# strukturag/libde265

Measured on NVIDIA H100. Metric: decoded frames/sec at 4K Main profile, bit-exact YUV; MC kernel HBM GB/s, higher is better.
Workload: dtype u8

## Files before the change

libde265_b200/csrc/engine.cu:

```cuda

#include <cuda_runtime.h>

#include <atomic>
#include <chrono>
#include <condition_variable>
#include <deque>
#include <exception>
#include <functional>
#include <mutex>
#include <string>
#include <sched.h>
#include <thread>
#include <cmath>
#include <cstdarg>
#include <cstdio>
#include <cstdlib>
#include <cstring>
#include <new>
#include <vector>

#include "b200hevc.h"
#include "dev_common.cuh"
#include "kernels_filter.cuh"
#include "kernels_mc.cuh"
// ... 204 lines not shown
    {
      std::lock_guard<std::mutex> lk(m);
      q.emplace_back(g, std::move(f));
      g->pending++;
    }
    cv.notify_one();
  }
  void wait(Group* g)
  {
    std::unique_lock<std::mutex> lk(m);
    done_cv.wait(lk, [g] { return g->pending == 0; });
  }
  void run(std::function<void()> f) { run(&own, std::move(f)); }
  void wait() { wait(&own); }
  ~HostPool()
  {
    {
      std::lock_guard<std::mutex> lk(m);
      stop = true;
    }
    cv.notify_all();
    for (auto& t : th) t.join();
  }
};

#define B200_MAX_CTX 12
#define B200_MAX_PHYS (B200_MAX_SLOTS + 32)
#define B200_STAGE_SETS 40
struct PipeCtx {
  cudaStream_t stream = nullptr;
  Surface scratch;
  uint8_t* sync_buf = nullptr;
  size_t sync_cap = 0;
  cudaEvent_t tail = nullptr;
};

struct SlotSync {
  cudaEvent_t written = nullptr;
  int writer = -1;
  cudaEvent_t read[B200_MAX_CTX] = {};
  bool read_pending[B200_MAX_CTX] = {};
};

#define PLAN_PU_PARTS 4
#define PLAN_INTRA_PARTS 8
struct IntraPart {
  uint32_t i0 = 0, i1 = 0, task_base = 0;
  std::vector<uint32_t> intra_idx, task_of, task_first, task_cell, diag_cnt, diag_off, fill;
};

struct AsyncState;
struct b200_engine {
  int device = 0;
  std::atomic<size_t> stage_cap_hint{0};
  std::mutex issue_m;
  AsyncState* async = nullptr;
  PipeCtx ctx[B200_MAX_CTX];
  StagingSet stage_pool[B200_STAGE_SETS];
  unsigned next_stage = 0;
  int n_ctx = 1, next_ctx = 0;
  Surface slot[B200_MAX_PHYS];
  SlotSync ssync[B200_MAX_PHYS];
  int lmap[B200_MAX_SLOTS];
  int owner[B200_MAX_PHYS];
  int last_owner[B200_MAX_PHYS];
  bool rename = true;
// ... 363 lines not shown
}

static int check_params(const b200_pic_params& p)
{
  if (p.width == 0 || p.height == 0) return set_err(B200_ERR_INVALID, "empty picture");
  if (p.log2_ctb_size < 4 || p.log2_ctb_size > 6) return set_err(B200_ERR_INVALID, "log2_ctb_size %d", p.log2_ctb_size);
  if (p.dst_slot >= B200_MAX_SLOTS) return set_err(B200_ERR_INVALID, "dst_slot %d", p.dst_slot);
  if (p.chroma_format_idc > 1) return set_err(B200_ERR_UNSUPPORTED, "chroma_format_idc %d: the device path implements 4:0:0 and 4:2:0", p.chroma_format_idc);
  if (p.bit_depth_luma < 8 || p.bit_depth_luma > 12 || p.bit_depth_chroma < 8 || p.bit_depth_chroma > 12)
    return set_err(B200_ERR_UNSUPPORTED, "bit depth %d/%d (8..12 supported)", p.bit_depth_luma, p.bit_depth_chroma);
  if ((p.bit_depth_luma > 8) != (p.bit_depth_chroma > 8)) return set_err(B200_ERR_UNSUPPORTED, "mixed 8-bit / high-bit-depth planes");
  if ((p.width & 7) || (p.height & 7)) return set_err(B200_ERR_INVALID, "picture size must be a multiple of the minimum CB size (8)");
  return B200_OK;
}

static DevPic make_devpic(const b200_pic_params& p, const Surface& cur, const Surface& out)
{
  DevPic d{};
  d.w = p.width; d.h = p.height;
  d.cw = cur.cw; d.ch = cur.ch;
  d.bd_y = p.bit_depth_luma; d.bd_c = p.bit_depth_chroma;
  d.log2ctb = p.log2_ctb_size;
  const int S = 1 << d.log2ctb;
  d.wctb = (p.width + S - 1) / S; d.hctb = (p.height + S - 1) / S;
  d.w4 = (p.width + 3) / 4; d.h4 = (p.height + 3) / 4;
  d.w8 = (p.width + 7) / 8; d.h8 = (p.height + 7) / 8;
  d.chroma = p.chroma_format_idc;
  d.cb_qp_off = p.pps_cb_qp_offset; d.cr_qp_off = p.pps_cr_qp_offset;
  d.flags = p.flags;
  for (int c = 0; c < 3; c++) { d.cur[c] = cur.plane[c]; d.out[c] = out.plane[c]; d.pitch[c] = cur.pitch[c]; }
  return d;
}

static size_t sync_sao_offset(const b200_pic_params& p)
{
  const size_t cw4 = p.chroma_format_idc ? (size_t)((p.width / 2 + 3) / 4) : 0, ch4 = p.chroma_format_idc ? (size_t)((p.height / 2 + 3) / 4) : 0;
  return (256 + (size_t)((p.width + 3) / 4) * ((p.height + 3) / 4) + 2 * cw4 * ch4 + 255) & ~(size_t)255;
}

template <typename P>
static int launch_picture(b200_engine* en, PipeCtx& cx, const PicLayout& L, const DevPic& dp, const RefTable& refs, const uint8_t* dbase)
{
  cudaStream_t st = cx.stream;
  const size_t* off = L.off;
  const int n_tiles = L.n_tiles;
  const bool run_deblock = L.run_deblock, run_sao = L.run_sao;
  if (en->timing) CU(cudaEventRecord(en->ev[1], st));
  if (n_tiles > 0) {
    if (sizeof(P) == 1 && !en->mc_legacy) {
      MctMaps maps;
      memset(&maps, 0, sizeof(maps));
      int n = 0;
      for (int i = 0; i < B200_MAX_SLOTS; i++) {
        maps.index_of_slot[i] = -1;
        if (!((L.ref_mask >> i) & 1) || !refs.plane[i][0] || !en->slot[en->lmap[i]].has_tm) continue;
        if (n == MCT_MAX_REFS) return set_err(B200_ERR_UNSUPPORTED, "picture references more than %d DPB slots", MCT_MAX_REFS);
        for (int k = 0; k < 2; k++) { maps.luma[k][n] = en->slot[en->lmap[i]].tm_luma[k]; maps.chroma[k][n] = en->slot[en->lmap[i]].tm_chroma[k]; }
        maps.index_of_slot[i] = (int8_t)n++;
        maps.valid_slots |= 1u << i;
      }
      const uint32_t* tw = (const uint32_t*)(dbase + off[12]);
      TL("mc", (k_inter_pred_tma<<<std::min(L.n_batches, en->num_sms * en->mc_ctas), MCT_CTA_THREADS, sizeof(MctShared), st>>>(
                   dp, maps, (const b200_pu*)(dbase + off[0]), (const b200_weight_entry*)(dbase + off[1]), tw, tw + n_tiles, L.n_batches)));
    } else if (sizeof(P) == 1)
      k_inter_pred8<<<std::min((n_tiles + MC8_UNITS_PER_CTA - 1) / MC8_UNITS_PER_CTA, en->num_sms * 5), MC8_WARPS * 32, 0, st>>>(dp, refs, (const b200_pu*)(dbase + off[0]), (const b200_weight_entry*)(dbase + off[1]),
                                                         (const uint32_t*)(dbase + off[12]), n_tiles);
    else
      k_inter_pred<P><<<(n_tiles + 3) / 4, 128, 0, st>>>(dp, refs, (const b200_pu*)(dbase + off[0]), (const b200_weight_entry*)(dbase + off[1]),
                                                           (const uint32_t*)(dbase + off[12]), n_tiles);
    en->launches++;
  }
  if (en->timing) CU(cudaEventRecord(en->ev[2], st));
  if ((L.n_a > 0 || L.n_b > 0) && L.params.stop_after_stage != B200_STAGE_INTER_PRED) {
    ReconArgs ra;
    ra.tus = (const b200_tu*)(dbase + off[2]);
    ra.coeffs = (const b200_coeff*)(dbase + off[5]);
    ra.scaling = L.has_scaling ? dbase + off[11] : nullptr;
    ra.ticket = (unsigned int*)cx.sync_buf;
    ra.region = en->region;
    ra.poll_ns = en->poll_ns;
    ra.err = en->intra_err;
    ra.err_host = en->intra_err_host;
    ra.spin_limit_ns = en->spin_limit_ns;
    const size_t cw4 = (size_t)((dp.cw + 3) / 4), ch4 = (size_t)((dp.ch + 3) / 4);
    ra.pend[0] = cx.sync_buf + 256;
    ra.pend[1] = ra.pend[0] + (size_t)dp.w4 * dp.h4;
    ra.pend[2] = ra.pend[1] + cw4 * ch4;
    ra.pend_w[0] = dp.w4;
    ra.pend_w[1] = ra.pend_w[2] = (int)cw4;
    ra.mark_list = nullptr;
    ra.n_mark = 0;
    if (L.n_b > 0) CU(cudaMemsetAsync(cx.sync_buf, 0, 256 + (size_t)dp.w4 * dp.h4 + 2 * cw4 * ch4, st));
    if (L.n_a > 0) {
      ra.list = (const uint32_t*)(dbase + off[3]);
      ra.n_list = L.n_a;
      ra.n_listw = L.n_aw;
      ra.n_list8 = L.n_a8;
      if (L.n_b > 0) {
        ra.mark_list = (const uint32_t*)(dbase + off[4]);
        ra.n_mark = L.n_b;
      }
      const int items = L.n_aw + (L.n_a8 + 3) / 4 + (L.n_a - L.n_aw - L.n_a8 + 31) / 32;
      TL("residual", (k_residual<P><<<std::min((items + RC_WARPS - 1) / RC_WARPS, en->num_sms * 4), RC_THREADS, 0, st>>>(dp, ra)));
      en->launches++;
    }
    ra.trace = nullptr;
    if (L.n_b > 0) {
      unsigned long long* trace_dev = nullptr;
      const char* trace_path = getenv("B200_TRACE_INTRA");
      if (trace_path && L.n_task > 0) {
        CU(cudaMalloc(&trace_dev, sizeof(unsigned long long) * RC_TRACE_WORDS * (size_t)L.n_task));
        CU(cudaMemsetAsync(trace_dev, 0, sizeof(unsigned long long) * RC_TRACE_WORDS * (size_t)L.n_task, st));
        ra.trace = trace_dev;
      }
      ra.list = (const uint32_t*)(dbase + off[4]);
      ra.n_list = L.n_b;
      if (L.n_a == 0) {
        TL("mark", (k_mark_pending<<<(L.n_b + 255) / 256, 256, 0, st>>>(ra)));
        en->launches++;
      }
      ra.task_start = (const uint32_t*)(dbase + off[13]);
      ra.n_task = L.n_task;
      int grid = (L.n_task + RC_WARPS - 1) / RC_WARPS;
      const bool background = L.ref_mask == 0 && en->n_ctx > 1;
      int cap = background ? (en->intra_i_grid ? en->intra_i_grid : en->num_sms) : en->num_sms * en->intra_ctas;
// ... 6 lines not shown
        std::vector<unsigned long long> h(RC_TRACE_WORDS * (size_t)L.n_task);
        std::vector<uint32_t> tasks((size_t)L.n_task + 1 + (size_t)L.n_b);
        CU(cudaStreamSynchronize(st));
        CU(cudaMemcpy(h.data(), trace_dev, h.size() * sizeof(unsigned long long), cudaMemcpyDeviceToHost));
        CU(cudaMemcpy(tasks.data(), ra.task_start, ((size_t)L.n_task + 1) * sizeof(uint32_t), cudaMemcpyDeviceToHost));
        CU(cudaMemcpy(tasks.data() + L.n_task + 1, ra.list, (size_t)L.n_b * sizeof(uint32_t), cudaMemcpyDeviceToHost));
        cudaFree(trace_dev);
        if (FILE* f = fopen(trace_path, "ab")) {
          const unsigned long long n[2] = {(unsigned long long)L.n_task, (unsigned long long)L.n_b};
          fwrite(n, sizeof(n), 1, f);
          fwrite(h.data(), sizeof(unsigned long long), h.size(), f);
          fwrite(tasks.data(), sizeof(uint32_t), tasks.size(), f);
          fclose(f);
        }
      }
    }
  }
  if (en->timing) CU(cudaEventRecord(en->ev[3], st));
  FilterArgs fa;
  fa.bs_map = dbase + off[8];
  fa.qp_map = (const int8_t*)(dbase + off[9]);
  fa.nofilt_map = dbase + off[10];
  fa.slices = (const b200_slice_info*)(dbase + off[6]);
  fa.ctbs = (const b200_ctb_info*)(dbase + off[7]);
  if (run_deblock) {
    const int nseg = ((dp.w4 + 1) / 2) * dp.h4 > dp.w4 * ((dp.h4 + 1) / 2) ? ((dp.w4 + 1) / 2) * dp.h4 : dp.w4 * ((dp.h4 + 1) / 2);
    dim3 grid((nseg + 127) / 128, dp.chroma ? 2 : 1);
    TL("deblock_v", (k_deblock<P, true><<<grid, 128, 0, st>>>(dp, fa)));
    TL("deblock_h", (k_deblock<P, false><<<grid, 128, 0, st>>>(dp, fa)));
    en->launches += 2;
  }
  if (en->timing) CU(cudaEventRecord(en->ev[4], st));
  if (run_sao) {
    uint16_t* avail = (uint16_t*)(cx.sync_buf + sync_sao_offset(L.params));
    fa.sao_avail = avail;
    const bool sao8 = sizeof(P) == 1 && dp.log2ctb >= 5 && !en->sao_legacy;
    if (!sao8) {
      TL("sao_prep", (k_sao_prep<<<(2 * dp.wctb * dp.hctb + 127) / 128, 128, 0, st>>>(dp, fa, avail)));
      en->launches++;
    }
    dim3 grid((dp.w / 8 + 127) / 128, dp.h, dp.chroma ? 3 : 1);
    if (sao8) {
      Sao8Layout lay;
      lay.n_ctb = dp.wctb * dp.hctb;
      const int S = 1 << dp.log2ctb, rows_l = (32 >> (dp.log2ctb - 4)) * SAO8_R, rows_c = (32 >> (dp.log2ctb - 5)) * SAO8_R;
      lay.ipl = (S + rows_l - 1) / rows_l;
      lay.ipc = dp.chroma ? (S / 2 + rows_c - 1) / rows_c : 0;
      const int items = lay.n_ctb * (lay.ipl + 2 * lay.ipc);
      TL("sao", (k_sao8<<<(items + SAO8_WARPS - 1) / SAO8_WARPS, SAO8_WARPS * 32, 0, st>>>(dp, fa, lay)));
    } else {
      TL("sao", (k_sao<P><<<grid, 128, 0, st>>>(dp, fa)));
    }
    en->launches++;
  }
  if (en->timing) CU(cudaEventRecord(en->ev[5], st));
  CU(cudaGetLastError());
  return B200_OK;
}

static const int k_raw_sections[10] = {0, 1, 2, 5, 6, 7, 8, 9, 10, 11};
static const int k_list_sections[4] = {3, 4, 12, 13};

static int plan_begin(b200_engine* en, const b200_picture* pic, PicLayout* L, size_t* cap_total)
{
  const b200_pic_params& p = pic->params;
  int rc = check_params(p);
  if (rc) return rc;
// ... 662 lines not shown
  RefTable refs;
  memset(&refs, 0, sizeof(refs));
  for (int i = 0; i < B200_MAX_SLOTS; i++) {
    if (i == p.dst_slot || en->lmap[i] < 0) continue;
    const Surface& s = en->slot[en->lmap[i]];
    if (s.valid && s.w == p.width && s.h == p.height && s.chroma == p.chroma_format_idc && s.bd_y == p.bit_depth_luma && s.bd_c == p.bit_depth_chroma)
      for (int c = 0; c < 3; c++) refs.plane[i][c] = s.plane[c];
  }
  {
    const uint64_t geom = (uint64_t)p.width | ((uint64_t)p.height << 16) | ((uint64_t)p.chroma_format_idc << 32) |
                          ((uint64_t)bytes_per_sample(p.bit_depth_luma) << 34) | ((uint64_t)bytes_per_sample(p.bit_depth_chroma) << 36);
    if (en->pool_geom && en->pool_geom != geom) {
      for (int c = 0; c < B200_MAX_CTX; c++) CU(cudaStreamSynchronize(en->ctx[c].stream));
      for (int ph = 0; ph < B200_MAX_PHYS; ph++)
        if (en->owner[ph] < 0 && en->slot[ph].plane[0] && !same_geometry(en->slot[ph], p)) surface_free(en->slot[ph]);
    }
    en->pool_geom = geom;
  }
  int dst_phys = phys_for_write(en, p.dst_slot, k, p);
  if (dst_phys < 0) {
    return set_err(B200_ERR_NOMEM, "no free picture surface");
  }
  Surface& dst = en->slot[dst_phys];
  int rc = surface_ensure(dst, p, cx.stream);
  if (rc) return rc;
  Surface* cur = &dst;
  if (L.run_sao) {
    rc = surface_ensure(cx.scratch, p, cx.stream);
    if (rc) return rc;
    cur = &cx.scratch;
  }
  {
    const size_t n_ctb = (size_t)((p.width + (1 << p.log2_ctb_size) - 1) >> p.log2_ctb_size) * ((p.height + (1 << p.log2_ctb_size) - 1) >> p.log2_ctb_size);
    const size_t need = sync_sao_offset(p) + 2 * n_ctb * sizeof(uint16_t);
    if (cx.sync_cap < need) {
      if (cx.sync_buf) { CU(cudaStreamSynchronize(cx.stream)); cudaFree(cx.sync_buf); }
      cx.sync_buf = nullptr;
      CU(cudaMalloc(&cx.sync_buf, need));
      cx.sync_cap = need;
    }
  }
  cudaStream_t st = cx.stream;
  en->ev = en->timing ? &en->tev[(size_t)(en->tcount % TIMING_RING) * 7] : nullptr;
  if (en->timing) CU(cudaEventRecord(en->ev[0], st));
  if (upload_from && L.direct) {
    for (int i : k_raw_sections)
      if (L.raw_sz[i]) CU(cudaMemcpyAsync(dbase + L.off[i], L.raw_src[i], L.raw_sz[i], cudaMemcpyHostToDevice, st));
    if (L.total > L.raw_total) CU(cudaMemcpyAsync(dbase + L.raw_total, upload_from + L.raw_total, L.total - L.raw_total, cudaMemcpyHostToDevice, st));
  } else if (upload_from) {
    CU(cudaMemcpyAsync(dbase, upload_from, L.total, cudaMemcpyHostToDevice, st));
  }
  if (prof) tseg[1] = now();
  rc = order_before(en, k, L, dst_phys);
  if (rc) return rc;
  if (prof) tseg[2] = now();
  const DevPic dp = make_devpic(p, *cur, dst);
  if (p.bit_depth_luma > 8) rc = launch_picture<uint16_t>(en, cx, L, dp, refs, dbase);
  else rc = launch_picture<uint8_t>(en, cx, L, dp, refs, dbase);
  if (rc) return rc;
  if (prof) tseg[3] = now();
  if (en->tl_path) tl_begin(en, st, "extend", L.params.poc, k);
  launch_extend_borders(dst, st);
  if (en->tl_path) tl_end(en, st);
  en->launches++;
  CU(cudaGetLastError());
  if (en->timing) { CU(cudaEventRecord(en->ev[6], st)); en->tcount++; }
  rc = order_after(en, k, L, dst_phys);
  if (rc) return rc;
  dst.valid = true;
  if (prof) {
    tseg[4] = now();
// ... 548 lines not shown
```

libde265_b200/csrc/kernels_recon.cuh:

```cuda
#pragma once
#include "dev_common.cuh"
#include "kernels_residual.cuh"

#define RC_WARPS 8
#define RC_THREADS (RC_WARPS * 32)
#define RC_GSTRIDE 34
#define RC_TILE_STRIDE 40
#define RC_BLK (33 * RC_TILE_STRIDE + 8)
#define RC_FULL 0xffffffffu
#define RC_TRACE_WORDS 8

struct ReconArgs {
  const b200_tu* tus;
  const uint32_t* list;
  int n_list;
  int poll_ns;
  int region;
  int n_listw, n_list8;
  const uint32_t* task_start;
  int n_task;
  const b200_coeff* coeffs;
  const uint8_t* scaling;
  unsigned int* ticket;
  unsigned long long* trace;
  uint8_t* pend[3];
  int pend_w[3];
  const uint32_t* mark_list;
  int n_mark;
  unsigned int* err;
  unsigned int* err_host;
  unsigned long long spin_limit_ns;
};

struct ResidualSmem {
  int16_t coef[RC_WARPS][32 * RC_GSTRIDE];
  int16_t g[RC_WARPS][32 * RC_GSTRIDE];
  ResTables tb;
};

template <typename P>
struct IntraSmem {
  P blk[RC_WARPS][RC_BLK];
  int16_t coef[RC_WARPS][32 * RC_GSTRIDE];
  int16_t g[RC_WARPS][32 * RC_GSTRIDE];
  res_t res[RC_WARPS][32 * 32];
  P border[RC_WARPS][2][4 * 32 + 4];
  b200_tu tu_s[RC_WARPS][16];
  ResTables tb;
};

template <typename P, bool TO_RES>
__device__ void tu_residual(const b200_tu& tu, const b200_coeff* co, const uint8_t* __restrict__ scaling, P* dst, int dstride, res_t* res,
                            int bd, int16_t* coefT, int16_t* g, const ResTables& tb, int lane)
{
  const int log2 = tu.log2_size, nT = 1 << log2, n = tu.n_coeff;
  const int flags = tu.flags;
  const bool special = flags & (B200_TU_BYPASS | B200_TU_TSKIP);
  const Dequant dq = dequant_setup(tu, scaling, bd);
  int max_row = 0, max_col = 0;
// ... 272 lines not shown
      if (bfilt) {
        if (mode == 26 && x == 0) v = clip_bd(B(1) + ((B(-1 - y) - B(0)) >> 1), bd);
        if (mode == 10 && y == 0) v = clip_bd(B(-1) + ((B(1 + x) - B(0)) >> 1), bd);
      }
      px[p] = v;
    }
  }
  __syncwarp();
#pragma unroll
  for (int p = 0; p < NP; p++) {
    const int o = lane + 32 * p, x = o & (nT - 1), y = (o >> LOG2) & (nT - 1);
    if (o < nT * nT) {
      int v = px[p];
      if (res) v = clip_bd(v + res[o], bd);
      dst[x + y * ts] = (P)v;
    }
  }
  __syncwarp();
}

__device__ __forceinline__ bool intra_fast_ok(const b200_tu& tu)
{
  const int g = 1 << (tu.log2_size - 2);
  const uint64_t need = ((1ull << g) - 1) | (1ull << B200_AVAIL_CORNER_BIT) | (((1ull << g) - 1) << B200_AVAIL_TOP_BIT0);
  if ((tu.avail & need) != need) return false;
  if (g == 2) {
    const unsigned bl = (unsigned)(tu.avail >> 2) & 3, tr = (unsigned)(tu.avail >> (B200_AVAIL_TOP_BIT0 + 2)) & 3;
    if (bl == 2 || tr == 2) return false;
  }
  return true;
}

template <typename P>
__device__ void tu_intra_large(const b200_tu& tu, const P* gsrc, int gstride, P* dst, int bd, int bd_luma, uint32_t pic_flags, bool filter_plane,
                               P* b0mem, P* b1mem, int lane)
{
  const int log2 = tu.log2_size, nT = 1 << log2, mode = tu.intra_mode, cidx = tu.cidx, dstride = nT;
  const uint64_t avail = tu.avail;
  P* b0 = b0mem + 2 * 32 + 2;
  P* b1 = b1mem + 2 * 32 + 2;
  const int total = 4 * nT + 1;
  {
    constexpr int MAXC = 5;
    int v[MAXC];
    bool av[MAXC];
#pragma unroll
    for (int c5 = 0; c5 < MAXC; c5++) {
      const int s = 32 * c5 + lane, i = s - 2 * nT;
      av[c5] = false;
      v[c5] = 0;
      if (s < total) {
        const P* addr;
        if (i < 0) { const int r = -i - 1; av[c5] = (avail >> (r >> 2)) & 1; addr = gsrc - 1 + r * gstride; }
        else if (i == 0) { av[c5] = (avail >> B200_AVAIL_CORNER_BIT) & 1; addr = gsrc - 1 - gstride; }
        else { const int c = i - 1; av[c5] = (avail >> (B200_AVAIL_TOP_BIT0 + (c >> 2))) & 1; addr = gsrc + c - gstride; }
        if (av[c5]) v[c5] = (int)__ldcg(addr);
      }
    }
    int first_val = 1 << (bd - 1);
    bool any = false;
#pragma unroll
    for (int c5 = 0; c5 < MAXC; c5++) {
      const unsigned m = __ballot_sync(0xffffffffu, av[c5]);
      if (!any && m) { first_val = __shfl_sync(0xffffffffu, v[c5], __ffs(m) - 1); any = true; }
    }
    if (!any) {
      for (int s = lane; s < total; s += 32) b0[s - 2 * nT] = (P)(1 << (bd - 1));
    } else {
      int carry = first_val;
#pragma unroll
      for (int c5 = 0; c5 < MAXC; c5++) {
        if (32 * c5 < total) {
          const int s = 32 * c5 + lane, i = s - 2 * nT;
          const unsigned m = __ballot_sync(0xffffffffu, av[c5]);
          const unsigned below = m & ((2u << lane) - 1u);
          const int src = below ? 31 - __clz(below) : 0;
          const int sv = __shfl_sync(0xffffffffu, v[c5], src);
          const int outv = below ? sv : carry;
          if (s < total) b0[i] = (P)outv;
          carry = __shfl_sync(0xffffffffu, outv, 31);
        }
      }
    }
  }
  __syncwarp();
  const P* bsrc = b0;
  if (filter_plane && mode != 1) {
    const int d = min(abs(mode - 26), abs(mode - 10));
    const bool filt = d > ((nT == 8) ? 7 : (nT == 16) ? 1 : 0);
    if (filt) {
      const bool strong = (pic_flags & B200_PIC_STRONG_INTRA_SMOOTHING) && cidx == 0 && nT == 32 &&
// ... 47 lines not shown
    for (int s = lane; s <= 3 * nT; s += 32) {
      const int x = s - nT;
      const bool w = (x >= 0) ? (x <= nT || angle >= 0) : (project && x >= last);
      const int idx = (x >= 0) ? sgn * x : -sgn * ((x * inv + 128) >> 8);
      if (w) ref[x] = bsrc[idx];
    }
    __syncwarp();
    const bool bfilt = (cidx == 0 && nT < 32 && !(tu.flags & B200_TU_NO_BOUNDARY_FILTER) && (mode == 26 || mode == 10));
    for (int o = lane; o < nT * nT; o += 32) {
      const int x = o & (nT - 1), y = o >> log2;
      const int a = vert ? y : x, b = vert ? x : y;
      const int idx = ((a + 1) * angle) >> 5, fact = ((a + 1) * angle) & 31;
      int v = fact ? ((32 - fact) * (int)ref[b + idx + 1] + fact * (int)ref[b + idx + 2] + 16) >> 5 : (int)ref[b + idx + 1];
      if (bfilt) {
        if (mode == 26 && x == 0) v = clip_bd((int)bsrc[1] + (((int)bsrc[-1 - y] - (int)bsrc[0]) >> 1), bd);
        if (mode == 10 && y == 0) v = clip_bd((int)bsrc[-1] + (((int)bsrc[1 + x] - (int)bsrc[0]) >> 1), bd);
      }
      dst[x + y * dstride] = (P)v;
    }
  }
  __syncwarp();
}

template <typename P>
__device__ __forceinline__ void block_store(const P* blk, uint8_t* plane, int pitch, int x, int y, int nT, int lane)
{
  const int upr = nT * (int)sizeof(P) / 4;
  for (int o = lane; o < nT * upr; o += 32) {
    const int r = o / upr, u = o % upr;
    *reinterpret_cast<uint32_t*>(plane + (size_t)(y + r) * pitch + (size_t)x * sizeof(P) + 4 * u) = reinterpret_cast<const uint32_t*>(blk + r * nT)[u];
  }
}

template <typename P>
__global__ void __launch_bounds__(RC_THREADS) k_residual(DevPic pic, ReconArgs args)
{
  __shared__ ResidualSmem sm;
  const int tid = threadIdx.x, warp = tid >> 5, lane = tid & 31;
  for (int i = tid; i < (int)(sizeof(ResTables) / 4); i += RC_THREADS) reinterpret_cast<uint32_t*>(&sm.tb)[i] = reinterpret_cast<const uint32_t*>(&c_res)[i];
  for (int i = blockIdx.x * RC_THREADS + tid; i < args.n_mark; i += gridDim.x * RC_THREADS) {
    const b200_tu tu = args.tus[args.mark_list[i]];
    const int c = tu.cidx, n4u = 1 << (tu.log2_size - 2);
    uint8_t* p = args.pend[c] + (tu.y >> 2) * args.pend_w[c] + (tu.x >> 2);
    for (int j = 0; j < n4u; j++)
      for (int k = 0; k < n4u; k++) p[j * args.pend_w[c] + k] = 1;
  }
  __syncthreads();
  const int n4 = args.n_list - args.n_listw - args.n_list8;
  const int Ww = args.n_listw, W8 = (args.n_list8 + 3) >> 2, W4 = (n4 + 31) >> 5;
  uint32_t* scratch = reinterpret_cast<uint32_t*>(sm.coef[warp]);
  for (int wi = blockIdx.x * RC_WARPS + warp; wi < Ww + W8 + W4; wi += gridDim.x * RC_WARPS) {
    if (wi < Ww) {
      const b200_tu tu = args.tus[args.list[wi]];
      const int c = tu.cidx, nT = 1 << tu.log2_size;
      P* dst = row_ptr<P>(pic.cur[c], pic.pitch[c], tu.y) + tu.x;
      const int dstride = pic.pitch[c] / (int)sizeof(P);
      if (tu.flags & B200_TU_PCM) {
        for (int i = lane; i < tu.n_coeff; i += 32) {
          const b200_coeff co = args.coeffs[tu.coeff_off + i];
          dst[(co.pos & (nT - 1)) + (co.pos >> tu.log2_size) * dstride] = (P)(uint16_t)co.level;
        }
      } else {
        tu_residual<P, false>(tu, args.coeffs + tu.coeff_off, args.scaling, dst, dstride, nullptr, c ? pic.bd_c : pic.bd_y, sm.coef[warp], sm.g[warp],
                              sm.tb, lane);
      }
    } else if (wi < Ww + W8) {
// ... 16 lines not shown
                            sm.tb);
      }
    }
    __syncwarp();
  }
}

__global__ void k_mark_pending(ReconArgs args)
{
  const int idx = blockIdx.x * blockDim.x + threadIdx.x;
  if (idx >= args.n_list) return;
  const b200_tu tu = args.tus[args.list[idx]];
  const int c = tu.cidx, n4 = 1 << (tu.log2_size - 2);
  uint8_t* p = args.pend[c] + (tu.y >> 2) * args.pend_w[c] + (tu.x >> 2);
  for (int j = 0; j < n4; j++)
    for (int i = 0; i < n4; i++) p[j * args.pend_w[c] + i] = 1;
}

__device__ __forceinline__ void dep_units_of(const b200_tu& tu, int rx, int ry, int span, unsigned& left, bool& corner, unsigned& top)
{
  const int half = 1 << (tu.log2_size - 1);
  const int ux0 = (tu.x - rx) >> 2, uy0 = (tu.y - ry) >> 2;
  const uint64_t avail = tu.avail;
  const unsigned gm = (half >= 32) ? 0xffffffffu : ((1u << half) - 1u), sm = (1u << span) - 1u;
  const bool cb = (avail >> B200_AVAIL_CORNER_BIT) & 1;
  if (ux0 == 0) {
    left |= (((unsigned)avail & gm) << uy0) & sm;
    if (cb) { if (uy0 == 0) corner = true; else left |= 1u << (uy0 - 1); }
  } else if (uy0 == 0 && cb) {
    top |= 1u << (ux0 - 1);
  }
  if (uy0 == 0) top |= (((unsigned)(avail >> B200_AVAIL_TOP_BIT0) & gm) << ux0) & sm;
}

__device__ __forceinline__ unsigned ld_acquire_u8(const uint8_t* p)
{
  unsigned v;
  asm volatile("ld.acquire.gpu.global.u8 %0, [%1];" : "=r"(v) : "l"(p) : "memory");
  return v;
}
__device__ __forceinline__ void st_relaxed_u8(uint8_t* p, unsigned v) { asm volatile("st.relaxed.gpu.global.u8 [%0], %1;" ::"l"(p), "r"(v) : "memory"); }

template <typename P>
__global__ void __launch_bounds__(RC_THREADS, 3) k_intra(DevPic pic, ReconArgs args)
{
  extern __shared__ __align__(16) uint8_t smem_raw[];
  IntraSmem<P>& sm = *reinterpret_cast<IntraSmem<P>*>(smem_raw);
  const int tid = threadIdx.x, warp = tid >> 5, lane = tid & 31;
  for (int i = tid; i < (int)(sizeof(ResTables) / 4); i += RC_THREADS) reinterpret_cast<uint32_t*>(&sm.tb)[i] = reinterpret_cast<const uint32_t*>(&c_res)[i];
  __syncthreads();
  b200_tu* tus = sm.tu_s[warp];
  res_t* res = sm.res[warp];
  P* blk = sm.blk[warp];
  for (;;) {
    unsigned t = 0;
    if (lane == 0) t = atomicAdd(args.ticket, 1u);
    t = __shfl_sync(RC_FULL, t, 0);
    if (t >= (unsigned)args.n_task) return;
    unsigned tr_c = 0;
    auto tr_time = [&](int w) {
      if (args.trace && lane == 0) {
        unsigned long long g;
        asm volatile("mov.u64 %0, %%globaltimer;" : "=l"(g));
        args.trace[(unsigned long long)RC_TRACE_WORDS * t + w] = g;
      }
    };
    auto tr_cycles = [&](int w) {
      if (args.trace && lane == 0) {
        const unsigned c = (unsigned)clock();
        if (w >= 0) args.trace[(unsigned long long)RC_TRACE_WORDS * t + w] += c - tr_c;
        tr_c = c;
      }
    };
    tr_time(0);
    tr_cycles(-1);
    const uint32_t first = args.task_start[t], count = min(args.task_start[t + 1] - first, 16u);
    if (lane < (int)count) tus[lane] = args.tus[args.list[first + lane]];
    __syncwarp();
    const b200_tu tu0 = tus[0];
    const int G0 = args.region >> (tu0.cidx ? 1 : 0);
    const bool region = (1 << tu0.log2_size) <= min(G0, 8);
    unsigned seg_starts;
    {
      const int mc = (lane < (int)count) ? tus[lane].cidx : -1, pc = (lane > 0 && lane < (int)count) ? tus[lane - 1].cidx : -1;
      seg_starts = __ballot_sync(RC_FULL, lane < (int)count && (lane == 0 || mc != pc));
    }
    {
      const bool mine = lane < (int)count;
      const b200_tu& mytu = tus[mine ? lane : 0];
      const int l2 = mytu.log2_size, sz = mine ? 1 << (2 * l2) : 0;
      const int mybd = mytu.cidx ? pic.bd_c : pic.bd_y;
      int incl = sz;
#pragma unroll
      for (int d = 1; d < 16; d <<= 1) {
        const int up = __shfl_up_sync(RC_FULL, incl, d);
        if (lane >= d) incl += up;
      }
      const int my_rbase = incl - sz;
      const bool cbf = mine && (mytu.flags & B200_TU_CBF);
      const unsigned m8 = __ballot_sync(RC_FULL, cbf && l2 == 3), mw = __ballot_sync(RC_FULL, cbf && l2 > 3);
      uint32_t* scratch = reinterpret_cast<uint32_t*>(sm.coef[warp]);
      if (cbf && l2 == 2) res4_lane<P, true>(mytu, args.coeffs + mytu.coeff_off, args.scaling, nullptr, 0, res + my_rbase, mybd, scratch, lane, sm.tb);
      __syncwarp();
      for (unsigned rem = m8; rem;) {
        const int q = lane >> 3;
        const unsigned idx = __fns(rem, 0, q + 1);
        const bool active = idx < 32u;
        const b200_tu& tu = tus[active ? idx : 0];
        const int rb = __shfl_sync(RC_FULL, my_rbase, active ? idx : 0);
        res8_quarter<P, true>(active, tu, args.coeffs + tu.coeff_off, args.scaling, nullptr, 0, res + rb, tu.cidx ? pic.bd_c : pic.bd_y, scratch + q * 64,
                              lane & 7, sm.tb);
#pragma unroll
        for (int k = 0; k < 4; k++) rem &= rem - 1;
      }
      for (unsigned rem = mw; rem; rem &= rem - 1) {
        const int idx = __ffs(rem) - 1;
        const b200_tu& tu = tus[idx];
        const int rb = __shfl_sync(RC_FULL, my_rbase, idx);
        tu_residual<P, true>(tu, args.coeffs + tu.coeff_off, args.scaling, nullptr, 0, res + rb, tu.cidx ? pic.bd_c : pic.bd_y, sm.coef[warp], sm.g[warp],
                             sm.tb, lane);
      }
    }
    tr_cycles(3);
    for (unsigned ss = seg_starts; ss; ss &= ss - 1) {
      const int s0 = __ffs(ss) - 1, s1 = (ss & (ss - 1)) ? __ffs(ss & (ss - 1)) - 1 : (int)count;
      const b200_tu& ts0 = tus[s0];
      const int c = ts0.cidx, G = args.region >> (c ? 1 : 0);
      const int rx = region ? ts0.x & ~(G - 1) : ts0.x, ry = region ? ts0.y & ~(G - 1) : ts0.y;
      const int span = region ? (2 * G) >> 2 : (1 << ts0.log2_size) >> 1;
      unsigned left = 0, top = 0;
      bool corner = false;
      if (lane >= s0 && lane < s1) dep_units_of(tus[lane], rx, ry, span, left, corner, top);
      left = __reduce_or_sync(RC_FULL, left);
      top = __reduce_or_sync(RC_FULL, top);
      corner = __any_sync(RC_FULL, corner);
      const int pw = args.pend_w[c];
      const uint8_t* pend = args.pend[c] + (ry >> 2) * pw + (rx >> 2);
      const uint8_t* f = nullptr;
      if (lane < span) { if ((left >> lane) & 1) f = pend + lane * pw - 1; }
      else if (lane == span) { if (corner) f = pend - pw - 1; }
      else if (lane - span - 1 < span) { if ((top >> (lane - span - 1)) & 1) f = pend - pw + (lane - span - 1); }
      const uint8_t* f2 = nullptr;
      if (span == 16 && lane == 0 && ((top >> 15) & 1)) f2 = pend - pw + 15;
      unsigned ns = 32, spins = 0;
      unsigned long long t_wait0 = 0;
      for (;;) {
        const bool busy = (f && ld_acquire_u8(f)) || (f2 && ld_acquire_u8(f2));
        if (!__any_sync(RC_FULL, busy)) break;
        __nanosleep(ns);
        if (ns < (unsigned)args.poll_ns) ns *= 2;
        else if ((++spins & 63u) == 0) {
          unsigned long long now;
          asm volatile("mov.u64 %0, %%globaltimer;" : "=l"(now));
          if (!t_wait0) t_wait0 = now;
          bool give_up = now - t_wait0 > args.spin_limit_ns || *(volatile unsigned int*)args.err != 0;
          give_up = __shfl_sync(RC_FULL, give_up, 0);
          if (give_up) {
            if (lane == 0) {
              atomicCAS(args.err, 0u, t + 1);
              *(volatile unsigned int*)args.err_host = t + 1;
              __threadfence_system();
            }
            break;
          }
        }
      }
    }
    __syncwarp();
    tr_time(1);
    tr_cycles(4);

    if (!region) {
      const int c = tu0.cidx, bd = c ? pic.bd_c : pic.bd_y;
      const bool filter_plane = !(pic.flags & B200_PIC_INTRA_SMOOTHING_OFF) && (c == 0 || pic.chroma == 3);
      const int nT = 1 << tu0.log2_size;
      const int gstride = pic.pitch[c] / (int)sizeof(P);
      const P* gsrc = row_ptr<P>(pic.cur[c], pic.pitch[c], tu0.y) + tu0.x;
      tu_intra_large<P>(tu0, gsrc, gstride, blk, bd, pic.bd_y, pic.flags, filter_plane, sm.border[warp][0], sm.border[warp][1], lane);
      if (tu0.flags & B200_TU_CBF) {
        for (int o = lane; o < nT * nT; o += 32) blk[o] = (P)clip_bd((int)blk[o] + res[o], bd);
        __syncwarp();
      }
      tr_cycles(6);
      block_store<P>(blk, pic.cur[c], pic.pitch[c], tu0.x, tu0.y, nT, lane);
    } else {
      int rbase = 0;
      for (unsigned ss = seg_starts; ss; ss &= ss - 1) {
        const int s0 = __ffs(ss) - 1, s1 = (ss & (ss - 1)) ? __ffs(ss & (ss - 1)) - 1 : (int)count;
        const b200_tu& ts0 = tus[s0];
        const int c = ts0.cidx, bd = c ? pic.bd_c : pic.bd_y, G = args.region >> (c ? 1 : 0);
        const int rx = ts0.x & ~(G - 1), ry = ts0.y & ~(G - 1);
        const bool filter_plane = !(pic.flags & B200_PIC_INTRA_SMOOTHING_OFF) && (c == 0 || pic.chroma == 3);
        const int pwid = c ? pic.cw : pic.w, phei = c ? pic.ch : pic.h;
        int covered = 0;
        for (int i = s0; i < s1; i++) covered += 1 << (2 * tus[i].log2_size);
        const int TS = RC_TILE_STRIDE;
        P* tile = blk + TS + 4;
        const int gw = min(G, pwid - rx), gh = min(G, phei - ry);
        const bool full = (gw == G) && (gh == G);
        tr_cycles(-1);
        const bool interior = covered < gw * gh;
        constexpr int NW = 2 * (int)sizeof(P);
        const int wpr = G * (int)sizeof(P) / 4;
        uint32_t in_w[NW];
        if (interior && full) {
#pragma unroll
          for (int k = 0; k < NW; k++) {
            const int o = lane + 32 * k;
            if (o < G * wpr) in_w[k] = __ldcg(reinterpret_cast<const uint32_t*>(row_ptr<P>(pic.cur[c], pic.pitch[c], ry + o / wpr) + rx) + o % wpr);
          }
        }
        const int xt0 = lane - 1, xt1 = lane + 31;
        const bool top0 = ry > 0 && xt0 < 2 * G && rx + xt0 >= 0 && rx + xt0 < pwid;
        const bool top1 = ry > 0 && xt1 < 2 * G && rx + xt1 < pwid;
        const bool left = rx > 0 && lane < 2 * G && ry + lane < phei;
        P top_s0, top_s1, left_s;
        if (top0) top_s0 = __ldcg(row_ptr<P>(pic.cur[c], pic.pitch[c], ry - 1) + rx + xt0);
        if (top1) top_s1 = __ldcg(row_ptr<P>(pic.cur[c], pic.pitch[c], ry - 1) + rx + xt1);
        if (left) left_s = __ldcg(row_ptr<P>(pic.cur[c], pic.pitch[c], ry + lane) + rx - 1);
        if (interior && full) {
#pragma unroll
          for (int k = 0; k < NW; k++) {
            const int o = lane + 32 * k;
            if (o < G * wpr) reinterpret_cast<uint32_t*>(tile + (o / wpr) * TS)[o % wpr] = in_w[k];
          }
        } else if (interior) {
          for (int o = lane; o < gw * gh; o += 32) {
            const int x = o % gw, y = o / gw;
            tile[y * TS + x] = __ldcg(row_ptr<P>(pic.cur[c], pic.pitch[c], ry + y) + rx + x);
          }
        }
        if (top0) tile[-TS + xt0] = top_s0;
        if (top1) tile[-TS + xt1] = top_s1;
        if (left) tile[lane * TS - 1] = left_s;
        __syncwarp();
        tr_cycles(5);
        for (int i = s0; i < s1; i++) {
          const b200_tu& tu = tus[i];
          P* tdst = tile + (tu.y - ry) * TS + (tu.x - rx);
          const res_t* tres = (tu.flags & B200_TU_CBF) ? res + rbase : nullptr;
          if (!intra_fast_ok(tu)) tu_intra_small<P>(tu, tdst, TS, bd, filter_plane, tres, lane);
          else if (tu.log2_size == 2) tu_intra_fast<P, 2>(tu, tdst, TS, bd, filter_plane, tres, lane);
          else tu_intra_fast<P, 3>(tu, tdst, TS, bd, filter_plane, tres, lane);
          rbase += 1 << (2 * tu.log2_size);
        }
        tr_cycles(6);
        if (full) {
          const int wpr = G * (int)sizeof(P) / 4;
          for (int o = lane; o < G * wpr; o += 32) {
            const int y = o / wpr, u = o % wpr;
            reinterpret_cast<uint32_t*>(row_ptr<P>(pic.cur[c], pic.pitch[c], ry + y) + rx)[u] = reinterpret_cast<const uint32_t*>(tile + y * TS)[u];
          }
        } else {
          for (int o = lane; o < gw * gh; o += 32) {
            const int x = o % gw, y = o / gw;
            row_ptr<P>(pic.cur[c], pic.pitch[c], ry + y)[rx + x] = tile[y * TS + x];
          }
        }
        __syncwarp();
      }
    }
    __syncwarp();
    if (lane < (int)count) {
      asm volatile("fence.release.gpu;" ::: "memory");
      const b200_tu& tu = tus[lane];
      const int n4 = 1 << (tu.log2_size - 2), pw = args.pend_w[tu.cidx];
      uint8_t* pend = args.pend[tu.cidx] + (tu.y >> 2) * pw + (tu.x >> 2);
      for (int j = 0; j < n4; j++)
        for (int i = 0; i < n4; i++) st_relaxed_u8(pend + j * pw + i, 0);
    }
    __syncwarp();
    tr_time(2);
    if (args.trace && lane == 0)
      args.trace[(unsigned long long)RC_TRACE_WORDS * t + 7] = count | ((unsigned long long)tu0.cidx << 8) | ((unsigned long long)tu0.log2_size << 16);
  }
}
```

Measured before the change: 2884.

## Replace per-TU pending-flag clears with tagged edge mailboxes in intra wavefront

Intra-prediction warps used to poll byte pending flags with acquire loads and clear them after each TU with a release fence. Now each finished block publishes its bottom row and right column as tagged 64-bit words into per-region mailboxes, so a dependent warp takes its neighbour samples straight from the mailbox once the tag matches. This removes the flag-clear and fence path and the re-read of neighbours from the picture. The tile interior is fetched with cp.async, which can overlap the wait. The cost is a larger sync buffer, extra stores for the edge data, and a periodic full memset when the tag wraps; correctness now depends on the tag and layout bookkeeping.

```diff
diff --git a/libde265_b200/csrc/engine.cu b/libde265_b200/csrc/engine.cu
--- a/libde265_b200/csrc/engine.cu
+++ b/libde265_b200/csrc/engine.cu
@@ -260,6 +260,7 @@
   Surface scratch;
   uint8_t* sync_buf = nullptr;
   size_t sync_cap = 0;
+  uint32_t tag = 0;
   cudaEvent_t tail = nullptr;
 };
 
@@ -689,10 +690,38 @@
   return d;
 }
 
-static size_t sync_sao_offset(const b200_pic_params& p)
-{
-  const size_t cw4 = p.chroma_format_idc ? (size_t)((p.width / 2 + 3) / 4) : 0, ch4 = p.chroma_format_idc ? (size_t)((p.height / 2 + 3) / 4) : 0;
-  return (256 + (size_t)((p.width + 3) / 4) * ((p.height + 3) / 4) + 2 * cw4 * ch4 + 255) & ~(size_t)255;
+struct SyncLayout {
+  size_t pend[3], pend_end, mbox0, hrow[3], vcol[3], mbox1, sao;
+  int pend_w[3], hrow_w[3], vcol_h[3];
+};
+static SyncLayout sync_layout(const b200_pic_params& p, int region)
+{
+  SyncLayout s;
+  const int bpw = p.bit_depth_luma > 8 ? 2 : 4;
+  int w[3], h[3];
+  w[0] = p.width; h[0] = p.height;
+  w[1] = w[2] = p.chroma_format_idc ? p.width / 2 : 0;
+  h[1] = h[2] = p.chroma_format_idc ? p.height / 2 : 0;
+  size_t o = 256;
+  for (int c = 0; c < 3; c++) {
+    s.pend[c] = o;
+    s.pend_w[c] = (w[c] + 3) / 4;
+    o += (size_t)s.pend_w[c] * ((h[c] + 3) / 4);
+  }
+  s.pend_end = o;
+  o = s.mbox0 = (o + 7) & ~(size_t)7;
+  for (int c = 0; c < 3; c++) {
+    const int G = region >> (c ? 1 : 0);
+    s.hrow_w[c] = (w[c] + bpw - 1) / bpw;
+    s.vcol_h[c] = (h[c] + bpw - 1) / bpw;
+    s.hrow[c] = o;
+    o += 8 * (size_t)(h[c] / G) * s.hrow_w[c];
+    s.vcol[c] = o;
+    o += 8 * (size_t)(w[c] / G) * s.vcol_h[c];
+  }
+  s.mbox1 = o;
+  s.sao = (o + 255) & ~(size_t)255;
+  return s;
 }
 
 template <typename P>
@@ -739,15 +768,23 @@
     ra.err = en->intra_err;
     ra.err_host = en->intra_err_host;
     ra.spin_limit_ns = en->spin_limit_ns;
-    const size_t cw4 = (size_t)((dp.cw + 3) / 4), ch4 = (size_t)((dp.ch + 3) / 4);
-    ra.pend[0] = cx.sync_buf + 256;
-    ra.pend[1] = ra.pend[0] + (size_t)dp.w4 * dp.h4;
-    ra.pend[2] = ra.pend[1] + cw4 * ch4;
-    ra.pend_w[0] = dp.w4;
-    ra.pend_w[1] = ra.pend_w[2] = (int)cw4;
+    const SyncLayout sl = sync_layout(L.params, en->region);
+    for (int c = 0; c < 3; c++) {
+      ra.pend[c] = cx.sync_buf + sl.pend[c];
+      ra.pend_w[c] = sl.pend_w[c];
+      ra.hrow[c] = (unsigned long long*)(cx.sync_buf + sl.hrow[c]);
+      ra.vcol[c] = (unsigned long long*)(cx.sync_buf + sl.vcol[c]);
+      ra.hrow_w[c] = sl.hrow_w[c];
+      ra.vcol_h[c] = sl.vcol_h[c];
+    }
+    if (++cx.tag == 0) {
+      CU(cudaMemsetAsync(cx.sync_buf, 0, cx.sync_cap, st));
+      cx.tag = 1;
+    }
+    ra.tag = cx.tag;
     ra.mark_list = nullptr;
     ra.n_mark = 0;
-    if (L.n_b > 0) CU(cudaMemsetAsync(cx.sync_buf, 0, 256 + (size_t)dp.w4 * dp.h4 + 2 * cw4 * ch4, st));
+    if (L.n_b > 0) CU(cudaMemsetAsync(cx.sync_buf, 0, sl.pend_end, st));
     if (L.n_a > 0) {
       ra.list = (const uint32_t*)(dbase + off[3]);
       ra.n_list = L.n_a;
@@ -820,7 +857,7 @@
   }
   if (en->timing) CU(cudaEventRecord(en->ev[4], st));
   if (run_sao) {
-    uint16_t* avail = (uint16_t*)(cx.sync_buf + sync_sao_offset(L.params));
+    uint16_t* avail = (uint16_t*)(cx.sync_buf + sync_layout(L.params, en->region).sao);
     fa.sao_avail = avail;
     const bool sao8 = sizeof(P) == 1 && dp.log2ctb >= 5 && !en->sao_legacy;
     if (!sao8) {
@@ -1549,11 +1586,12 @@
   }
   {
     const size_t n_ctb = (size_t)((p.width + (1 << p.log2_ctb_size) - 1) >> p.log2_ctb_size) * ((p.height + (1 << p.log2_ctb_size) - 1) >> p.log2_ctb_size);
-    const size_t need = sync_sao_offset(p) + 2 * n_ctb * sizeof(uint16_t);
+    const size_t need = sync_layout(p, en->region).sao + 2 * n_ctb * sizeof(uint16_t);
     if (cx.sync_cap < need) {
       if (cx.sync_buf) { CU(cudaStreamSynchronize(cx.stream)); cudaFree(cx.sync_buf); }
       cx.sync_buf = nullptr;
       CU(cudaMalloc(&cx.sync_buf, need));
+      CU(cudaMemsetAsync(cx.sync_buf, 0, need, cx.stream));
       cx.sync_cap = need;
     }
   }
diff --git a/libde265_b200/csrc/kernels_recon.cuh b/libde265_b200/csrc/kernels_recon.cuh
--- a/libde265_b200/csrc/kernels_recon.cuh
+++ b/libde265_b200/csrc/kernels_recon.cuh
@@ -25,6 +25,10 @@
   unsigned long long* trace;
   uint8_t* pend[3];
   int pend_w[3];
+  unsigned long long* hrow[3];
+  unsigned long long* vcol[3];
+  int hrow_w[3], vcol_h[3];
+  unsigned tag;
   const uint32_t* mark_list;
   int n_mark;
   unsigned int* err;
@@ -363,8 +367,7 @@
 }
 
 template <typename P>
-__device__ void tu_intra_large(const b200_tu& tu, const P* gsrc, int gstride, P* dst, int bd, int bd_luma, uint32_t pic_flags, bool filter_plane,
-                               P* b0mem, P* b1mem, int lane)
+__device__ void tu_intra_large(const b200_tu& tu, P* dst, int bd, int bd_luma, uint32_t pic_flags, bool filter_plane, P* b0mem, P* b1mem, int lane)
 {
   const int log2 = tu.log2_size, nT = 1 << log2, mode = tu.intra_mode, cidx = tu.cidx, dstride = nT;
   const uint64_t avail = tu.avail;
@@ -381,13 +384,13 @@
       av[c5] = false;
       v[c5] = 0;
       if (s < total) {
-        const P* addr;
-        if (i < 0) { const int r = -i - 1; av[c5] = (avail >> (r >> 2)) & 1; addr = gsrc - 1 + r * gstride; }
-        else if (i == 0) { av[c5] = (avail >> B200_AVAIL_CORNER_BIT) & 1; addr = gsrc - 1 - gstride; }
-        else { const int c = i - 1; av[c5] = (avail >> (B200_AVAIL_TOP_BIT0 + (c >> 2))) & 1; addr = gsrc + c - gstride; }
-        if (av[c5]) v[c5] = (int)__ldcg(addr);
-      }
-    }
+        if (i < 0) av[c5] = (avail >> ((-i - 1) >> 2)) & 1;
+        else if (i == 0) av[c5] = (avail >> B200_AVAIL_CORNER_BIT) & 1;
+        else av[c5] = (avail >> (B200_AVAIL_TOP_BIT0 + ((i - 1) >> 2))) & 1;
+        if (av[c5]) v[c5] = (int)b0[i];
+      }
+    }
+    __syncwarp();
     int first_val = 1 << (bd - 1);
     bool any = false;
 #pragma unroll
@@ -501,6 +504,43 @@
   }
 }
 
+__device__ __forceinline__ void cp_async4(void* smem, const void* gmem)
+{
+  asm volatile("cp.async.ca.shared.global [%0], [%1], 4;" ::"r"((unsigned)__cvta_generic_to_shared(smem)), "l"(gmem) : "memory");
+}
+
+__device__ __forceinline__ unsigned long long ld_relaxed_b64(const unsigned long long* p)
+{
+  unsigned long long v;
+  asm volatile("ld.relaxed.gpu.global.b64 %0, [%1];" : "=l"(v) : "l"(p));
+  return v;
+}
+__device__ __forceinline__ void st_relaxed_b64(unsigned long long* p, unsigned long long v)
+{
+  asm volatile("st.relaxed.gpu.global.b64 [%0], %1;" ::"l"(p), "l"(v) : "memory");
+}
+
+template <typename P>
+__device__ __forceinline__ void publish_edges(const ReconArgs& args, int c, const P* src, int sstride, int x0, int y0, int w, int h, int G, int lane)
+{
+  constexpr int BPW = 4 / (int)sizeof(P);
+  const int nr = (h >= G) ? w / BPW : 0, wc = h / BPW, nc = (w / G) * wc;
+  const unsigned long long tag = (unsigned long long)args.tag << 32;
+  for (int o = lane; o < nr + nc; o += 32) {
+    if (o < nr) {
+      const uint32_t d = *reinterpret_cast<const uint32_t*>(src + (h - 1) * sstride + o * BPW);
+      st_relaxed_b64(args.hrow[c] + (size_t)((y0 + h) / G - 1) * args.hrow_w[c] + x0 / BPW + o, tag | d);
+    } else {
+      const int a = (o - nr) / wc, j = (o - nr) - a * wc;
+      const P* s = src + (j * BPW) * sstride + (a + 1) * G - 1;
+      uint32_t d = 0;
+#pragma unroll
+      for (int k = 0; k < BPW; k++) d |= (uint32_t)s[k * sstride] << (8 * (int)sizeof(P) * k);
+      st_relaxed_b64(args.vcol[c] + (size_t)(x0 / G + a) * args.vcol_h[c] + y0 / BPW + j, tag | d);
+    }
+  }
+}
+
 template <typename P>
 __global__ void __launch_bounds__(RC_THREADS) k_residual(DevPic pic, ReconArgs args)
 {
@@ -583,14 +623,6 @@
   }
   if (uy0 == 0) top |= (((unsigned)(avail >> B200_AVAIL_TOP_BIT0) & gm) << ux0) & sm;
 }
-
-__device__ __forceinline__ unsigned ld_acquire_u8(const uint8_t* p)
-{
-  unsigned v;
-  asm volatile("ld.acquire.gpu.global.u8 %0, [%1];" : "=r"(v) : "l"(p) : "memory");
-  return v;
-}
-__device__ __forceinline__ void st_relaxed_u8(uint8_t* p, unsigned v) { asm volatile("st.relaxed.gpu.global.u8 [%0], %1;" ::"l"(p), "r"(v) : "memory"); }
 
 template <typename P>
 __global__ void __launch_bounds__(RC_THREADS, 3) k_intra(DevPic pic, ReconArgs args)
@@ -629,12 +661,12 @@
     if (lane < (int)count) tus[lane] = args.tus[args.list[first + lane]];
     __syncwarp();
     const b200_tu tu0 = tus[0];
-    const int G0 = args.region >> (tu0.cidx ? 1 : 0);
-    const bool region = (1 << tu0.log2_size) <= min(G0, 8);
+    if (args.trace && lane == 0)
+      args.trace[(unsigned long long)RC_TRACE_WORDS * t + 7] = count | ((unsigned long long)tu0.cidx << 8) | ((unsigned long long)tu0.log2_size << 16);
     unsigned seg_starts;
     {
       const int mc = (lane < (int)count) ? tus[lane].cidx : -1, pc = (lane > 0 && lane < (int)count) ? tus[lane - 1].cidx : -1;
-      seg_starts = __ballot_sync(RC_FULL, lane < (int)count && (lane == 0 || mc != pc));
+      seg_starts = __ballot_sync(RC_FULL, lane == (int)count || (lane < (int)count && (lane == 0 || mc != pc)));
     }
     {
       const bool mine = lane < (int)count;
@@ -673,119 +705,151 @@
       }
     }
     tr_cycles(3);
-    for (unsigned ss = seg_starts; ss; ss &= ss - 1) {
-      const int s0 = __ffs(ss) - 1, s1 = (ss & (ss - 1)) ? __ffs(ss & (ss - 1)) - 1 : (int)count;
+    int rbase = 0;
+    for (unsigned ss = seg_starts; ss & (ss - 1); ss &= ss - 1) {
+      tr_cycles(-1);
+      const int s0 = __ffs(ss) - 1, s1 = __ffs(ss & (ss - 1)) - 1;
       const b200_tu& ts0 = tus[s0];
-      const int c = ts0.cidx, G = args.region >> (c ? 1 : 0);
+      const int c = ts0.cidx, bd = c ? pic.bd_c : pic.bd_y, G = args.region >> (c ? 1 : 0);
+      const bool region = (1 << ts0.log2_size) <= min(G, 8);
       const int rx = region ? ts0.x & ~(G - 1) : ts0.x, ry = region ? ts0.y & ~(G - 1) : ts0.y;
       const int span = region ? (2 * G) >> 2 : (1 << ts0.log2_size) >> 1;
+      const bool filter_plane = !(pic.flags & B200_PIC_INTRA_SMOOTHING_OFF) && (c == 0 || pic.chroma == 3);
       unsigned left = 0, top = 0;
       bool corner = false;
       if (lane >= s0 && lane < s1) dep_units_of(tus[lane], rx, ry, span, left, corner, top);
       left = __reduce_or_sync(RC_FULL, left);
       top = __reduce_or_sync(RC_FULL, top);
       corner = __any_sync(RC_FULL, corner);
+      constexpr int TS = RC_TILE_STRIDE;
+      P* const tile = blk + TS + 4;
+      P* const b0 = sm.border[warp][0] + 2 * 32 + 2;
+      P* const e_left = region ? tile - 1 : b0 - 1;
+      const int e_ls = region ? TS : -1;
+      P* const e_top = region ? tile - TS : b0 + 1;
+      const int pwid = c ? pic.cw : pic.w, phei = c ? pic.ch : pic.h;
+      const int gw = region ? min(G, pwid - rx) : 0, gh = region ? min(G, phei - ry) : 0;
+      const bool full = (gw == G) && (gh == G);
+      if (region) {
+        int covered = 0;
+        for (int i = s0; i < s1; i++) covered += 1 << (2 * tus[i].log2_size);
+        if (covered < gw * gh) {
+          const int wpr = gw * (int)sizeof(P) / 4;
+          for (int o = lane; o < wpr * gh; o += 32) {
+            const int y = o / wpr, u = o - y * wpr;
+            cp_async4(tile + y * TS + u * (4 / (int)sizeof(P)), row_ptr<P>(pic.cur[c], pic.pitch[c], ry + y) + rx + u * (4 / (int)sizeof(P)));
+          }
+        }
+      }
+      constexpr int BPW = 4 / (int)sizeof(P), UW = (int)sizeof(P);
       const int pw = args.pend_w[c];
       const uint8_t* pend = args.pend[c] + (ry >> 2) * pw + (rx >> 2);
-      const uint8_t* f = nullptr;
-      if (lane < span) { if ((left >> lane) & 1) f = pend + lane * pw - 1; }
-      else if (lane == span) { if (corner) f = pend - pw - 1; }
-      else if (lane - span - 1 < span) { if ((top >> (lane - span - 1)) & 1) f = pend - pw + (lane - span - 1); }
-      const uint8_t* f2 = nullptr;
-      if (span == 16 && lane == 0 && ((top >> 15) & 1)) f2 = pend - pw + 15;
-      unsigned ns = 32, spins = 0;
-      unsigned long long t_wait0 = 0;
-      for (;;) {
-        const bool busy = (f && ld_acquire_u8(f)) || (f2 && ld_acquire_u8(f2));
-        if (!__any_sync(RC_FULL, busy)) break;
-        __nanosleep(ns);
-        if (ns < (unsigned)args.poll_ns) ns *= 2;
-        else if ((++spins & 63u) == 0) {
-          unsigned long long now;
-          asm volatile("mov.u64 %0, %%globaltimer;" : "=l"(now));
-          if (!t_wait0) t_wait0 = now;
-          bool give_up = now - t_wait0 > args.spin_limit_ns || *(volatile unsigned int*)args.err != 0;
-          give_up = __shfl_sync(RC_FULL, give_up, 0);
-          if (give_up) {
-            if (lane == 0) {
-              atomicCAS(args.err, 0u, t + 1);
-              *(volatile unsigned int*)args.err_host = t + 1;
-              __threadfence_system();
+      const unsigned long long* vc = args.vcol[c] + (long long)(rx / G - 1) * args.vcol_h[c] + ry / BPW;
+      const unsigned long long* hr = args.hrow[c] + (long long)(ry / G - 1) * args.hrow_w[c] + rx / BPW;
+      auto unit = [&](int k, bool& is_left, int& u) -> bool {
+        const int v = lane + 32 * k;
+        is_left = v <= span;
+        u = is_left ? v - 1 : v - span - 1;
+        return is_left ? (u < 0 ? corner : (left >> u) & 1) : v <= 2 * span && ((top >> u) & 1);
+      };
+      auto mbox = [&](bool is_left, int u) { return (is_left ? vc : hr) + (4 * u) / BPW; };
+      auto stage = [&](bool is_left, int u, const uint32_t (&dd)[UW]) {
+#pragma unroll
+        for (int s = 0; s < 4; s++) {
+          const P smp = (P)(dd[(s * UW) >> 2] >> ((8 * (int)sizeof(P) * s) & 31));
+          if (!is_left) e_top[4 * u + s] = smp;
+          else if (u >= 0 || s == 3) e_left[(4 * u + s) * e_ls] = smp;
+        }
+      };
+      unsigned polling = 0;
+#pragma unroll
+      for (int k = 0; k < 2; k++) {
+        bool is_left;
+        int u;
+        if (unit(k, is_left, u)) {
+          const unsigned intra = __ldcg(is_left ? pend + u * pw - 1 : pend - pw + u);
+          uint32_t pd[UW], wd[UW];
+          bool ok = true;
+#pragma unroll
+          for (int i = 0; i < UW; i++) {
+            const unsigned long long w = ld_relaxed_b64(mbox(is_left, u) + i);
+            wd[i] = (uint32_t)w;
+            ok &= (unsigned)(w >> 32) == args.tag;
+            pd[i] = 0;
+          }
+          if (is_left) {
+            const P* col = row_ptr<P>(pic.cur[c], pic.pitch[c], ry + 4 * u) + rx - 1;
+#pragma unroll
+            for (int s = 0; s < 4; s++) pd[(s * UW) >> 2] |= (uint32_t)__ldcg(col + s * (pic.pitch[c] / (int)sizeof(P))) << ((8 * (int)sizeof(P) * s) & 31);
+          } else {
+            const uint32_t* row = reinterpret_cast<const uint32_t*>(row_ptr<P>(pic.cur[c], pic.pitch[c], ry - 1) + rx + 4 * u);
+#pragma unroll
+            for (int i = 0; i < UW; i++) pd[i] = __ldcg(row + i);
+          }
+          if (!intra) stage(is_left, u, pd);
+          else if (ok) stage(is_left, u, wd);
+          else polling |= 1u << k;
+        }
+      }
+      {
+        unsigned ns = 32, spins = 0;
+        unsigned long long t_wait0 = 0;
+        while (__any_sync(RC_FULL, polling != 0)) {
+          __nanosleep(ns);
+          if (ns < (unsigned)args.poll_ns) ns *= 2;
+          else if ((++spins & 63u) == 0) {
+            unsigned long long now;
+            asm volatile("mov.u64 %0, %%globaltimer;" : "=l"(now));
+            if (!t_wait0) t_wait0 = now;
+            bool give_up = now - t_wait0 > args.spin_limit_ns || *(volatile unsigned int*)args.err != 0;
+            give_up = __shfl_sync(RC_FULL, give_up, 0);
+            if (give_up) {
+              if (lane == 0) {
+                atomicCAS(args.err, 0u, t + 1);
+                *(volatile unsigned int*)args.err_host = t + 1;
+                __threadfence_system();
+              }
+              break;
             }
-            break;
           }
-        }
-      }
-    }
-    __syncwarp();
-    tr_time(1);
-    tr_cycles(4);
-
-    if (!region) {
-      const int c = tu0.cidx, bd = c ? pic.bd_c : pic.bd_y;
-      const bool filter_plane = !(pic.flags & B200_PIC_INTRA_SMOOTHING_OFF) && (c == 0 || pic.chroma == 3);
-      const int nT = 1 << tu0.log2_size;
-      const int gstride = pic.pitch[c] / (int)sizeof(P);
-      const P* gsrc = row_ptr<P>(pic.cur[c], pic.pitch[c], tu0.y) + tu0.x;
-      tu_intra_large<P>(tu0, gsrc, gstride, blk, bd, pic.bd_y, pic.flags, filter_plane, sm.border[warp][0], sm.border[warp][1], lane);
-      if (tu0.flags & B200_TU_CBF) {
-        for (int o = lane; o < nT * nT; o += 32) blk[o] = (P)clip_bd((int)blk[o] + res[o], bd);
-        __syncwarp();
-      }
-      tr_cycles(6);
-      block_store<P>(blk, pic.cur[c], pic.pitch[c], tu0.x, tu0.y, nT, lane);
-    } else {
-      int rbase = 0;
-      for (unsigned ss = seg_starts; ss; ss &= ss - 1) {
-        const int s0 = __ffs(ss) - 1, s1 = (ss & (ss - 1)) ? __ffs(ss & (ss - 1)) - 1 : (int)count;
-        const b200_tu& ts0 = tus[s0];
-        const int c = ts0.cidx, bd = c ? pic.bd_c : pic.bd_y, G = args.region >> (c ? 1 : 0);
-        const int rx = ts0.x & ~(G - 1), ry = ts0.y & ~(G - 1);
-        const bool filter_plane = !(pic.flags & B200_PIC_INTRA_SMOOTHING_OFF) && (c == 0 || pic.chroma == 3);
-        const int pwid = c ? pic.cw : pic.w, phei = c ? pic.ch : pic.h;
-        int covered = 0;
-        for (int i = s0; i < s1; i++) covered += 1 << (2 * tus[i].log2_size);
-        const int TS = RC_TILE_STRIDE;
-        P* tile = blk + TS + 4;
-        const int gw = min(G, pwid - rx), gh = min(G, phei - ry);
-        const bool full = (gw == G) && (gh == G);
-        tr_cycles(-1);
-        const bool interior = covered < gw * gh;
-        constexpr int NW = 2 * (int)sizeof(P);
-        const int wpr = G * (int)sizeof(P) / 4;
-        uint32_t in_w[NW];
-        if (interior && full) {
-#pragma unroll
-          for (int k = 0; k < NW; k++) {
-            const int o = lane + 32 * k;
-            if (o < G * wpr) in_w[k] = __ldcg(reinterpret_cast<const uint32_t*>(row_ptr<P>(pic.cur[c], pic.pitch[c], ry + o / wpr) + rx) + o % wpr);
+#pragma unroll
+          for (int k = 0; k < 2; k++) {
+            if (!((polling >> k) & 1)) continue;
+            bool is_left;
+            int u;
+            unit(k, is_left, u);
+            uint32_t wd[UW];
+            bool ok = true;
+#pragma unroll
+            for (int i = 0; i < UW; i++) {
+              const unsigned long long w = ld_relaxed_b64(mbox(is_left, u) + i);
+              wd[i] = (uint32_t)w;
+              ok &= (unsigned)(w >> 32) == args.tag;
+            }
+            if (ok) {
+              stage(is_left, u, wd);
+              polling &= ~(1u << k);
+            }
           }
         }
-        const int xt0 = lane - 1, xt1 = lane + 31;
-        const bool top0 = ry > 0 && xt0 < 2 * G && rx + xt0 >= 0 && rx + xt0 < pwid;
-        const bool top1 = ry > 0 && xt1 < 2 * G && rx + xt1 < pwid;
-        const bool left = rx > 0 && lane < 2 * G && ry + lane < phei;
-        P top_s0, top_s1, left_s;
-        if (top0) top_s0 = __ldcg(row_ptr<P>(pic.cur[c], pic.pitch[c], ry - 1) + rx + xt0);
-        if (top1) top_s1 = __ldcg(row_ptr<P>(pic.cur[c], pic.pitch[c], ry - 1) + rx + xt1);
-        if (left) left_s = __ldcg(row_ptr<P>(pic.cur[c], pic.pitch[c], ry + lane) + rx - 1);
-        if (interior && full) {
-#pragma unroll
-          for (int k = 0; k < NW; k++) {
-            const int o = lane + 32 * k;
-            if (o < G * wpr) reinterpret_cast<uint32_t*>(tile + (o / wpr) * TS)[o % wpr] = in_w[k];
-          }
-        } else if (interior) {
-          for (int o = lane; o < gw * gh; o += 32) {
-            const int x = o % gw, y = o / gw;
-            tile[y * TS + x] = __ldcg(row_ptr<P>(pic.cur[c], pic.pitch[c], ry + y) + rx + x);
-          }
-        }
-        if (top0) tile[-TS + xt0] = top_s0;
-        if (top1) tile[-TS + xt1] = top_s1;
-        if (left) tile[lane * TS - 1] = left_s;
-        __syncwarp();
-        tr_cycles(5);
+      }
+      asm volatile("cp.async.wait_all;" ::: "memory");
+      __syncwarp();
+      tr_time(1);
+      tr_cycles(4);
+      tr_cycles(5);
+
+      if (!region) {
+        const int nT = 1 << ts0.log2_size;
+        tu_intra_large<P>(ts0, blk, bd, pic.bd_y, pic.flags, filter_plane, sm.border[warp][0], sm.border[warp][1], lane);
+        if (ts0.flags & B200_TU_CBF) {
+          for (int o = lane; o < nT * nT; o += 32) blk[o] = (P)clip_bd((int)blk[o] + res[o], bd);
+          __syncwarp();
+        }
+        tr_cycles(6);
+        publish_edges<P>(args, c, blk, nT, ts0.x, ts0.y, nT, nT, G, lane);
+        block_store<P>(blk, pic.cur[c], pic.pitch[c], ts0.x, ts0.y, nT, lane);
+      } else {
         for (int i = s0; i < s1; i++) {
           const b200_tu& tu = tus[i];
           P* tdst = tile + (tu.y - ry) * TS + (tu.x - rx);
@@ -796,6 +860,7 @@
           rbase += 1 << (2 * tu.log2_size);
         }
         tr_cycles(6);
+        publish_edges<P>(args, c, tile, TS, rx, ry, gw, gh, G, lane);
         if (full) {
           const int wpr = G * (int)sizeof(P) / 4;
           for (int o = lane; o < G * wpr; o += 32) {
@@ -808,21 +873,9 @@
             row_ptr<P>(pic.cur[c], pic.pitch[c], ry + y)[rx + x] = tile[y * TS + x];
           }
         }
-        __syncwarp();
-      }
-    }
-    __syncwarp();
-    if (lane < (int)count) {
-      asm volatile("fence.release.gpu;" ::: "memory");
-      const b200_tu& tu = tus[lane];
-      const int n4 = 1 << (tu.log2_size - 2), pw = args.pend_w[tu.cidx];
-      uint8_t* pend = args.pend[tu.cidx] + (tu.y >> 2) * pw + (tu.x >> 2);
-      for (int j = 0; j < n4; j++)
-        for (int i = 0; i < n4; i++) st_relaxed_u8(pend + j * pw + i, 0);
-    }
-    __syncwarp();
+      }
+      __syncwarp();
+    }
     tr_time(2);
-    if (args.trace && lane == 0)
-      args.trace[(unsigned long long)RC_TRACE_WORDS * t + 7] = count | ((unsigned long long)tu0.cidx << 8) | ((unsigned long long)tu0.log2_size << 16);
-  }
-}
+  }
+}
```

Result: faster. 2918, median of 6 (+1.2%).
